# vr308/Generalised-Gaussian-Processes

Hardware: AMD Instinct MI355X
Metric: ELBO evals/sec (higher is better)
Workload: dtype f64

## Files before the change

### generalised-gaussian-processes_amd/_lib.py

```python
from __future__ import annotations

import ctypes as C
import os

HERE = os.path.dirname(os.path.abspath(__file__))
LIB_PATH = os.path.join(HERE, "csrc", "libsgp_hip.so")

SGP_ABI_VERSION = 3
SGP_MAX_DIM = 32
SGP_MAX_INDUCING = 4096
KERNEL_IDS = {"rbf": 0, "matern32": 1, "matern52": 2, "composite": 3}
LIKELIHOOD_IDS = {"gaussian": 0, "bernoulli": 1, "bernoulli_logit": 2, "poisson": 3}
SGPMC_LIK_OUT_LEN = 3
SGP_LIK_MULTICLASS_ROBUSTMAX = 4
SGP_MAX_CLASSES = 16
COMP_LEN = 33
OPT_CONTRACTION, OPT_ASM_OVERLAP, OPT_KFU_BUDGET_BYTES, OPT_COND_LIMIT, OPT_CU_BUDGET, OPT_TIMING, OPT_SHARED_DEVICE = range(7)
OUT_F, OUT_LOGMARG, OUT_TRACE, OUT_LOGDETB, OUT_QUAD, OUT_TRW, OUT_S2BAR, OUT_KAPPABAR, OUT_LEN = range(9)


class SgpLibraryError(RuntimeError):
    pass


class SgpStatusError(RuntimeError):
    def __init__(self, fn, status, text):
        super().__init__("%s returned %d: %s" % (fn, status, text))
        self.status = status


_vp, _i64, _i32, _dbl, _sz = C.c_void_p, C.c_int64, C.c_int, C.c_double, C.c_size_t
_dp = C.POINTER(C.c_double)
# ... 329 lines not shown
```

### generalised-gaussian-processes_amd/core.py

```python
from __future__ import annotations

import math

import torch

try:
    import torch.distributed as dist
except Exception:
    dist = None

from ._lib import COMP_LEN, OUT_F, OUT_LOGMARG, OUT_S2BAR, OUT_TRACE


class NotPositiveDefiniteError(RuntimeError):

    def __init__(self, info):
        super().__init__("matrix not positive definite: leading minor of order %d (1..M: Kuu, M+1..2M: B)" % info)
        self.info = info


class SgpTimeoutError(RuntimeError):

    def __init__(self):
        super().__init__("device time-out inside the dataflow Cholesky (SGP_INFO_TIMEOUT): outputs are invalid")
# ... 346 lines not shown
            self._allreduce_stats(packed, M)
            kw = {"want_cw": True} if factored else {}
            res = e.bound(Kuu, packed, s2, self.N, with_adjoints=with_adjoints, want_factors=want_factors, kuu_linv=linv,
                          result=result, whitened=True, **kw)
            if rep:
                e.streaming_error_report(None, 1, self._trace_buf(), sf2, s2, self.N, M, result)
                res["reported"] = True
            res.update(packed=packed, kfu=None, t_keep=t_keep, linv=linv)
            return res
        kfu = self._kfu_for(M) if with_adjoints else None
        gate = None
        guard = report
        trace = self._trace_buf() if guard and hasattr(e, "kuu_factor") else None
        overlap = (self.overlap_tail and hasattr(e, "kuu_factor") and e.device.type == "cuda"
                   and int(self.X.shape[0]) * M >= self.overlap_min_work)
        if overlap:
            main = torch.cuda.current_stream(e.device)
            side, (z_ready, ready), (Kuu, linv) = self._side_state(M)
            z_ready.record(main)
            side.wait_event(z_ready)
            e.kuu(Z, ls, sf2, self.jitter, self.kernel, out=Kuu, stream=side)
            e.kuu_factor(Kuu, info=result[2], trace_out=trace, out=linv, stream=side)
            ready.record(side)
            if (hasattr(e, "would_use_i8") and self.kernel != "composite" and int(self.X.shape[0]) >= 300 * M
                    and e.would_use_i8(int(self.X.shape[0]), M)):
                gate = ready
        try:
            packed = e.suffstats(self.X, self.y, Z, ls, sf2, self.kernel, kfu=kfu, **({"gate": gate} if gate is not None else {}))
            self._allreduce_stats(packed, M)
        finally:
            if overlap:
                main.wait_event(ready)
        if overlap:
            res = e.bound(Kuu, packed, s2, self.N, with_adjoints=with_adjoints, want_factors=want_factors, kuu_linv=linv,
                          result=result)
        elif guard and hasattr(e, "kuu_factor"):
            Kuu = e.kuu(Z, ls, sf2, self.jitter, self.kernel)
            linv, _ = e.kuu_factor(Kuu, info=result[2], trace_out=trace)
            res = e.bound(Kuu, packed, s2, self.N, with_adjoints=with_adjoints, want_factors=want_factors, kuu_linv=linv,
                          result=result)
        else:
            Kuu = e.kuu(Z, ls, sf2, self.jitter, self.kernel)
            res = e.bound(Kuu, packed, s2, self.N, with_adjoints=with_adjoints, want_factors=want_factors, result=result)
        if guard and trace is not None:
            e.streaming_error_report(packed, M + 1, trace, sf2, s2, self.N, M, result)
            res["reported"] = True
        res["packed"] = packed
        res["kfu"] = kfu
        return res

    def _pass2(self, res, Z, ls, sf2, s2, want_gz, g):
        e = self.engine
        if res.get("Cw") is not None:
            e.suffstats_bwd_factored(self.X, self.y, Z, ls, sf2, res["linv"], res["Cw"], s2, res["bbar"], -1.0 / (2.0 * float(s2)),
                                     self.kernel, want_gz=want_gz, out=g,
                                     **({"t_in": res["t_keep"]} if res.get("t_keep") is not None else {}))
        else:
            e.suffstats_bwd(self.X, self.y, Z, ls, sf2, res["Phibar"], res["bbar"], -1.0 / (2.0 * float(s2)),
                            self.kernel, want_gz=want_gz, out=g, kfu=res["kfu"])
            if res.get("Phibar_lo") is not None:
# ... 180 lines not shown
```

### generalised-gaussian-processes_amd/csrc/sgp_ctx.hip

```cpp
#include "sgp_common.hpp"
#include "sgp_ctx.hpp"
#include "sgp_stream.hpp"
#include <cstdlib>
#include <new>

namespace sgp {

static void ctx_init(Ctx& c, int device) {
  c.device = device;
  c.contraction = env_int("SGP_CONTRACTION", 1);
  if (c.contraction < 0 || c.contraction > 2) c.contraction = 1;
  c.asm_overlap = env_int("SGP_ASM_OVERLAP", 0);
  c.kfu_budget = KFU_BUDGET_DEFAULT;
  c.syrk_skip_upper = env_int("SGP_SYRK_SKIP_UPPER", 1);
  c.syrk_waves = env_int("SGP_SYRK_WAVES", 4);
  c.syrk_glds = env_int("SGP_SYRK_GLDS", 0);
  c.i8_prio = env_int("SGP_I8_PRIO", 0);
  c.shared_device = env_int("SGP_SHARED_DEVICE", 0) != 0 ? 1 : 0;
}

Ctx& default_ctx() {
  static Ctx* c = [] {
    Ctx* p = new Ctx();
    int dev = 0;
    if (hipGetDevice(&dev) != hipSuccess) dev = 0;
    ctx_init(*p, dev);
    return p;
  }();
  return *c;
}

static thread_local Ctx* t_cur = nullptr;
static thread_local Ctx* t_bound = nullptr;
// ... 51 lines not shown
      if (!(value >= 0.0)) return SGP_ERR_ARG;
      c.kfu_budget = value > 0.0 ? (size_t)value : KFU_BUDGET_DEFAULT;
      return SGP_OK;
    case SGP_OPT_COND_LIMIT:
      c.cond_limit = value >= 0.0 ? value : 1e13;
      return SGP_OK;
    case SGP_OPT_CU_BUDGET:
      c.cu_budget = value > 0.0 ? (int)value : 0;
      return SGP_OK;
    case SGP_OPT_TIMING:
      c.timing = value != 0.0 ? 1 : 0;
      return SGP_OK;
    case SGP_OPT_SHARED_DEVICE:
      c.shared_device = value != 0.0 ? 1 : 0;
      return SGP_OK;
    default:
      return SGP_ERR_ARG;
  }
}

extern "C" double sgp_ctx_get_option(const sgp_ctx* ctx, int option) {
  const Ctx& c = ctx ? *reinterpret_cast<const Ctx*>(ctx) : default_ctx();
  switch (option) {
    case SGP_OPT_CONTRACTION: return (double)c.contraction;
    case SGP_OPT_ASM_OVERLAP: return (double)c.asm_overlap;
    case SGP_OPT_KFU_BUDGET_BYTES: return (double)c.kfu_budget;
    case SGP_OPT_COND_LIMIT: return c.cond_limit;
    case SGP_OPT_CU_BUDGET: return (double)c.cu_budget;
    case SGP_OPT_TIMING: return (double)c.timing;
    case SGP_OPT_SHARED_DEVICE: return (double)c.shared_device;
    default: return -1.0;
  }
}

extern "C" void sgp_ctx_bind_thread(sgp_ctx* ctx) { sgp::bind_thread_ctx(ctx); }

extern "C" int sgp_ctx_device(const sgp_ctx* ctx) { return (ctx ? *reinterpret_cast<const Ctx*>(ctx) : default_ctx()).device; }

extern "C" void sgp_ctx_set_pass1_gate(sgp_ctx* ctx, void* hip_event) {
  (ctx ? *reinterpret_cast<Ctx*>(ctx) : default_ctx()).pass1_gate = (hipEvent_t)hip_event;
}

extern "C" int sgp_ctx_contraction_last(const sgp_ctx* ctx) {
  return (ctx ? *reinterpret_cast<const Ctx*>(ctx) : default_ctx()).contraction_used;
}
// ... 159 lines not shown
```

### generalised-gaussian-processes_amd/csrc/sgp_ctx.hpp

```cpp
#pragma once
#include <hip/hip_runtime.h>
#include <cstddef>
#include <cstdint>

namespace sgp {

constexpr int CTX_TIMING_SLOTS = 3;

struct Ctx {
  int device = 0;
  int contraction = 1;
  int asm_overlap = 0;
  size_t kfu_budget = 0;
  double cond_limit = 1e13;
  int cu_budget = 0;
  int timing = 0;
  int shared_device = 0;
  int syrk_skip_upper = 1, syrk_waves = 4, syrk_glds = 0, i8_prio = 0;
  int contraction_used = 0;
  hipEvent_t pass1_gate = nullptr;
  int64_t syrk_timed_rows = 0;
  hipEvent_t ev[CTX_TIMING_SLOTS][2] = {};
  int ev_ready = 0, ev_used[CTX_TIMING_SLOTS] = {0, 0, 0};
  hipStream_t side = nullptr;
  hipEvent_t ev_fork = nullptr, ev_join = nullptr;
};

Ctx& default_ctx();
Ctx& cur_ctx();

void bind_thread_ctx(void* ctx);

struct CtxScope {
  Ctx* prev;
  explicit CtxScope(void* ctx);
// ... 7 lines not shown
```

### generalised-gaussian-processes_amd/csrc/sgp_suffstats_fwd.hip

```cpp
#include "sgp_common.hpp"
#include "sgp_stream.hpp"
#include "sgp_dense.hpp"
#include "sgp_composite.hpp"
#include "sgp_ctx.hpp"
#include <cstdlib>

namespace sgp {

static_assert(TIMING_SLOTS == CTX_TIMING_SLOTS, "timing slots");
size_t stream_kfu_budget() { return cur_ctx().kfu_budget; }

void timing_begin(int slot, hipStream_t st) {
  Ctx& c = cur_ctx();
  if (!c.timing) return;
  if (!c.ev_ready) {
    bool ok = true;
    for (int s = 0; s < TIMING_SLOTS; ++s)
      for (int k = 0; k < 2; ++k) ok = (hipEventCreate(&c.ev[s][k]) == hipSuccess) && ok;
    if (!ok) return;
    c.ev_ready = 1;
  }
  if (hipEventRecord(c.ev[slot][0], st) != hipSuccess) c.ev_used[slot] = 0;
}
void timing_end(int slot, hipStream_t st) {
// ... 304 lines not shown
    split = (nsplit & ~7) + u / ntiles;
  }
  int ti = (int)((sqrt(8.0 * t + 1.0) - 1.0) * 0.5);
  while ((ti + 1) * (ti + 2) / 2 <= t) ++ti;
  while (ti * (ti + 1) / 2 > t) --ti;
  const int tj = t - ti * (ti + 1) / 2;
  int64_t c0, c1;
  split_range(smap, split, nchunks, c0, c1);
  double* out = slab + ((size_t)split * ntiles + t) * (TILE * TILE);
  if (ti == tj)
    syrk_tile<true, NW, GLDS, SKIP>(Ks, Kfu, Mp, c0, c1, ti * TILE, tj * TILE, accumulate, out);
  else
    syrk_tile<false, NW, GLDS, SKIP>(Ks, Kfu, Mp, c0, c1, ti * TILE, tj * TILE, accumulate, out);
}

__global__ __launch_bounds__(256) void reduce_phi_kernel(const double* __restrict__ slab, int nsplit, int ntiles,
                                                         int M, double scale, double* __restrict__ Phi) {
  __shared__ double tile[32][33];
  const int t = blockIdx.x;
  int bi = (int)((sqrt(8.0 * t + 1.0) - 1.0) * 0.5);
  while ((bi + 1) * (bi + 2) / 2 <= t) ++bi;
  while (bi * (bi + 1) / 2 > t) --bi;
  const int bj = t - bi * (bi + 1) / 2;
  const int tx = threadIdx.x & 31, ty = threadIdx.x >> 5;
  const int Ti = (bi * 32) / TILE, Tj = (bj * 32) / TILE;
  const int tileidx = Ti * (Ti + 1) / 2 + Tj;
  const double* base = slab + (size_t)tileidx * (TILE * TILE);
  const size_t sstride = (size_t)ntiles * (TILE * TILE);
#pragma unroll
  for (int k = 0; k < 4; ++k) {
    const int lr = ty + 8 * k;
    const int gi = bi * 32 + lr, gj = bj * 32 + tx;
    double s = 0.0;
    if (gi >= gj) {
      const size_t off = (size_t)(gi - Ti * TILE) * TILE + (gj - Tj * TILE);
#pragma unroll 8
      for (int sp = 0; sp < nsplit; ++sp) s += base[sp * sstride + off];
    }
    tile[lr][tx] = s * scale;
  }
  __syncthreads();
#pragma unroll
  for (int k = 0; k < 4; ++k) {
    const int lr = ty + 8 * k;
    const int gi = bi * 32 + lr, gj = bj * 32 + tx;
    if (gi < M && gj < M && gi >= gj) Phi[(size_t)gi * M + gj] = tile[lr][tx];
    const int mi = bj * 32 + lr, mj = bi * 32 + tx;
    if (mi < M && mj < M && mj > mi) Phi[(size_t)mi * M + mj] = tile[tx][lr];
  }
}

__global__ __launch_bounds__(256) void bpart_stage1_kernel(const double* __restrict__ bpart, int64_t nrb, int Mp, int G,
                                                           double* __restrict__ tmp) {
  __shared__ double part[4][64];
  const int col = blockIdx.x * 64 + (threadIdx.x & 63), w = threadIdx.x >> 6, g = blockIdx.y;
  double s = 0.0;
  for (int64_t rb = g + (int64_t)w * G; rb < nrb; rb += 4 * (int64_t)G) s += bpart[rb * Mp + col];
  part[w][threadIdx.x & 63] = s;
  __syncthreads();
  if (w == 0) {
    const int l = threadIdx.x;
    tmp[(size_t)g * Mp + col] = (part[0][l] + part[1][l]) + (part[2][l] + part[3][l]);
  }
}
// ... 4 lines not shown
                                                             double* __restrict__ yy, double* __restrict__ kappa) {
  const int m = blockIdx.x * 256 + threadIdx.x;
  if (m < M) {
    double s = 0.0;
#pragma unroll 8
    for (int g = 0; g < G; ++g) s += btmp[(size_t)g * Mp + m];
    b[m] = s * sf2;
  }
  if (blockIdx.x == 0) {
    __shared__ double red[4];
    double s = 0.0;
    for (int i = threadIdx.x; i < nyy; i += 256) s += yypart[i];
    s = block_sum256(s, red);
    if (threadIdx.x == 0) {
      *yy = s;
      *kappa = kappa_val;
    }
  }
}

template <int DP, int ROWS>
static void launch_assemble_rows(int kid, dim3 grid, hipStream_t st, const double* Xs, const double* ys, const double* Zs,
                                 int64_t row0, int64_t N, int M, int Mp, double* Kfu, double* bpart) {
  switch (kid) {
    case SGP_KERNEL_RBF: kfu_assemble_kernel<DP, SGP_KERNEL_RBF, ROWS><<<grid, 256, 0, st>>>(Xs, ys, Zs, row0, N, M, Mp, Kfu, bpart); break;
    case SGP_KERNEL_MATERN32: kfu_assemble_kernel<DP, SGP_KERNEL_MATERN32, ROWS><<<grid, 256, 0, st>>>(Xs, ys, Zs, row0, N, M, Mp, Kfu, bpart); break;
    default: kfu_assemble_kernel<DP, SGP_KERNEL_MATERN52, ROWS><<<grid, 256, 0, st>>>(Xs, ys, Zs, row0, N, M, Mp, Kfu, bpart); break;
  }
}
template <int DP>
// ... 110 lines not shown
                   double* b, double* yy, double* kappa, hipStream_t st) {
  bpart_stage1_kernel<<<dim3(p.Mp / 64, BRED_G), 256, 0, st>>>(bpart, p.Npad / ASM_ROWS * nparts, p.Mp, BRED_G, btmp);
  finalize_stats_kernel<<<(M + 255) / 256, 256, 0, st>>>(btmp, BRED_G, p.Mp, M, yypart, 256, sf2, sf2 * (double)N, b, yy, kappa);
}
template <typename Ws>
static void finish_b(const StreamPlan& p, const Ws& w, int nparts, double sf2, int64_t N, int M, double* b, double* yy, double* kappa,
                     hipStream_t st) {
  reduce_bparts(p, w.bpart, w.btmp, w.yypart, nparts, sf2, N, M, b, yy, kappa, st);
}
void reduce_slabs(const StreamPlan& p, const double* slab, int nslabs, int M, double scale, double* Phi, hipStream_t st) {
  const int nb32 = p.Mp / 32;
  reduce_phi_kernel<<<nb32 * (nb32 + 1) / 2, 256, 0, st>>>(slab, nslabs, p.ntiles, M, scale, Phi);
}
static void finish_stats(const StreamPlan& p, const FwdWs& w, int nslabs, int nparts, double sf2, int64_t N, int M, double* Phi, double* b,
                         double* yy, double* kappa, hipStream_t st) {
  reduce_slabs(p, w.slab, nslabs, M, sf2 * sf2, Phi, st);
  finish_b(p, w, nparts, sf2, N, M, b, yy, kappa, st);
}

__global__ __launch_bounds__(256) void tpart_kernel(const double* __restrict__ T, const double* __restrict__ ys, int64_t row0, int Mp,
                                                    double* __restrict__ bpart) {
  __shared__ double ysh[ASM_ROWS];
  const int64_t rbase = (int64_t)blockIdx.x * ASM_ROWS;
  ysh[threadIdx.x] = ys[row0 + rbase + threadIdx.x];
  __syncthreads();
  const int m = blockIdx.y * 256 + threadIdx.x;
  if (m >= Mp) return;
  const double* src = T + (size_t)rbase * Mp + m;
  double a0 = 0.0, a1 = 0.0, a2 = 0.0, a3 = 0.0;
#pragma unroll 2
// ... 470 lines not shown
```

### generalised-gaussian-processes_amd/csrc/sgp_tail.hip

```cpp
#include "sgp_dense.hpp"
#include "sgp_ctx.hpp"
#include "sgp_composite.hpp"
#include "sgp_stream.hpp"

namespace sgp {

template <int KID>
__global__ __launch_bounds__(256) void kuu_kernel(const double* __restrict__ Z, int64_t ldz, KernArgs ka, double jitter,
                                                  int M, double* __restrict__ Kuu) {
  const int64_t total = (int64_t)M * M;
  for (int64_t e = (int64_t)blockIdx.x * 256 + threadIdx.x; e < total; e += (int64_t)gridDim.x * 256) {
    const int i = (int)(e / M), j = (int)(e - (int64_t)i * M);
    double r2 = 0.0;
    for (int q = 0; q < ka.d; ++q) {
      const double df = (Z[i * ldz + q] - Z[j * ldz + q]) * ka.inv_ls[q];
      r2 = fma(df, df, r2);
    }
    double v = ka.sf2 * kprofile<KID>(r2);
    if (i == j) v += jitter;
    Kuu[e] = v;
  }
}

template <int KID>
// ... 121 lines not shown
        else g_ls[q] += -2.0 * ka.inv_ls[q] * s;
      }
    }
  }
  if (g_Z) {
    const int64_t total = (int64_t)M * d;
    for (int64_t e = (int64_t)blockIdx.x * 256 + threadIdx.x; e < total; e += (int64_t)gridDim.x * 256) {
      const int q = (int)(e % d);
      g_Z[e] += 4.0 * ka.inv_ls[q] * gzraw[e];
    }
  }
}

enum { SC_TRW = 0, SC_LOGDET = 1, SC_QQ = 2, SC_TRSP = 3, SC_BA = 4, SC_APA = 5, SC_N = 8 };

__global__ __launch_bounds__(256) void make_B_kernel(const double* __restrict__ W, int Mp, double inv_s2, double* __restrict__ Bm,
                                                     double* __restrict__ trW, double* __restrict__ zero_me, int nB,
                                                     const double* __restrict__ Li, const double* __restrict__ x, double* __restrict__ y) {
  if ((int)blockIdx.x >= nB) {
    const int row = ((int)blockIdx.x - nB) * 4 + (threadIdx.x >> 6), lane = threadIdx.x & 63;
    if (row >= Mp) return;
    double s = 0.0;
    for (int j = lane; j < Mp; j += 64) s = fma(Li[(int64_t)row * Mp + j], x[j], s);
    s = wave_sum(s);
    if (lane == 0) y[row] = s;
    return;
  }
  const int64_t total = (int64_t)Mp * Mp;
  for (int64_t e = (int64_t)blockIdx.x * 256 + threadIdx.x; e < total; e += (int64_t)nB * 256) {
    const int r = (int)(e / Mp), c = (int)(e - (int64_t)r * Mp);
    const double w = 0.5 * (W[e] + W[(int64_t)c * Mp + r]);
    Bm[e] = (r == c ? 1.0 : 0.0) + w * inv_s2;
    if (zero_me) zero_me[e] = 0.0;
  }
  if ((int)blockIdx.x == nB - 1) {
    __shared__ double red[4];
    double s = 0.0;
    for (int i = threadIdx.x; i < Mp; i += 256) s += W[(int64_t)i * Mp + i];
// ... 76 lines not shown
  out[SGP_OUT_LOGMARG] = logmarg;
  out[SGP_OUT_TRACE] = trace_term;
  out[SGP_OUT_LOGDETB] = logdetB;
  out[SGP_OUT_QUAD] = quad;
  out[SGP_OUT_TRW] = trW;
  if (with_adj) {
    const double s22 = s2 * s2;
    out[SGP_OUT_S2BAR] = -0.5 * (-trSP / s22 + Nd / s2 - *yy / s22 + 2.0 * ba / (s22 * s2) - aPa / (s22 * s22)
                                 - *kappa / s22 + trW / s22);
    out[SGP_OUT_KAPPABAR] = -1.0 / (2.0 * s2);
  } else {
    out[SGP_OUT_S2BAR] = 0.0;
    out[SGP_OUT_KAPPABAR] = 0.0;
  }
}
__global__ __launch_bounds__(256) void finalize_bound_kernel(FinalizeArgs a) {
  __shared__ double red[4];
  finalize_bound_body(a, red);
}

__global__ __launch_bounds__(1024) void adjoint_mid_kernel(const double* __restrict__ W, const double* __restrict__ Binv,
                                                           const double* __restrict__ g, const double* __restrict__ u,
                                                           const double* __restrict__ Li, int Mp, double s2, int nC,
                                                           double* __restrict__ CS, double* __restrict__ rows3, double* __restrict__ t) {
  __shared__ double part[16][64];
  const int b = blockIdx.x, lane = threadIdx.x & 63, wv = threadIdx.x >> 6;
  if (b < nC) {
    const int64_t total = (int64_t)Mp * Mp;
    const double is2 = 1.0 / s2, is22 = 1.0 / (s2 * s2);
    for (int64_t e = (int64_t)b * 1024 + threadIdx.x; e < total; e += (int64_t)nC * 1024) {
      const int r = (int)(e / Mp), c = (int)(e - (int64_t)r * Mp);
      const int64_t pt = (int64_t)c * Mp + r;
      const double w = 0.5 * (W[e] + W[pt]);
// ... 34 lines not shown
      s3 = fma(Li[(int64_t)(j + 48) * Mp + col], g[j + 48], s3);
    }
    for (; j < Mp; j += 16) s0 = fma(Li[(int64_t)j * Mp + col], g[j], s0);
    part[wv][lane] = (s0 + s1) + (s2_ + s3);
    __syncthreads();
    if (wv == 0) {
      double acc = 0.0;
#pragma unroll
      for (int k = 0; k < 16; ++k) acc += part[k][lane];
      t[col] = acc;
    }
  }
}
__global__ __launch_bounds__(256) void adjoint_out_kernel(const double* __restrict__ R, const double* __restrict__ t,
                                                          int Mp, int M, double s2, double* __restrict__ Phibar,
                                                          double* __restrict__ Kuubar, double* __restrict__ bbar, int nA, FinalizeArgs fin) {
  if ((int)blockIdx.x == nA) {
    __shared__ double red[4];
    finalize_bound_body(fin, red);
    return;
  }
  const int64_t total = (int64_t)M * M;
  const int64_t mm = (int64_t)Mp * Mp;
  const double h = 0.25 / s2;
  for (int64_t e = (int64_t)blockIdx.x * 256 + threadIdx.x; e < total; e += (int64_t)nA * 256) {
    const int r = (int)(e / M), c = (int)(e - (int64_t)r * M);
    const int64_t p = (int64_t)r * Mp + c, pt = (int64_t)c * Mp + r;
    Phibar[e] = h * (R[p] + R[pt]);
    Kuubar[e] = -0.25 * (R[mm + p] + R[mm + pt]);
  }
  const double is22 = 1.0 / (s2 * s2);
  if (blockIdx.x == 0)
    for (int i = threadIdx.x; i < M; i += 256) bbar[i] = t[i] * is22;
}
// ... 452 lines not shown
}

__global__ void streaming_bound_kernel(const double* __restrict__ tr, double sf2, double s2, double* __restrict__ est) {
  est[0] = 0x1p-53 * sf2 * sf2 * tr[0] / s2;
}
extern "C" int sgp_streaming_error_bound(const double* trace_inv, double sf2, double s2, double* est, sgp_stream_t stream) {
  if (!trace_inv || !est || !(s2 > 0.0) || !(sf2 > 0.0)) return SGP_ERR_ARG;
  streaming_bound_kernel<<<1, 1, 0, (hipStream_t)stream>>>(trace_inv, sf2, s2, est);
  return check_launch();
}

__global__ __launch_bounds__(256) void streaming_report_kernel(const double* __restrict__ diag, int64_t stride, int M,
                                                               const double* __restrict__ tr, double sf2, double s2, double n,
                                                               double* __restrict__ est) {
  __shared__ double red[4];
  double mx = 0.0;
  if (diag)
    for (int i = threadIdx.x; i < M; i += 256) mx = fmax(mx, diag[(int64_t)i * stride]);
#pragma unroll
  for (int o = 32; o > 0; o >>= 1) mx = fmax(mx, __shfl_xor(mx, o, 64));
  if ((threadIdx.x & 63) == 0) red[threadIdx.x >> 6] = mx;
  __syncthreads();
  if (threadIdx.x == 0) {
    const double ub = 0x1p-53 * sf2 * sf2 * tr[0] / s2;
    est[1] = ub;
    est[0] = diag ? 0x1p-53 * fmax(fmax(red[0], red[1]), fmax(red[2], red[3])) * tr[0] / (s2 * n) : ub;
  }
}
extern "C" int sgp_streaming_error_report(const double* diag, int64_t stride, const double* trace_inv, double sf2, double s2, int64_t N,
                                          int M, double* est, sgp_stream_t stream) {
  if (!trace_inv || !est || M <= 0 || N < 0 || !(s2 > 0.0) || !(sf2 > 0.0) || (diag && stride <= 0)) return SGP_ERR_ARG;
  if (M > SGP_MAX_INDUCING) return SGP_ERR_DIM;
  streaming_report_kernel<<<1, 256, 0, (hipStream_t)stream>>>(diag, stride, M, trace_inv, sf2, s2, N > 0 ? (double)N : 1.0, est);
  return check_launch();
}

extern "C" void sgp_set_cond_limit(double limit) { default_ctx().cond_limit = limit >= 0.0 ? limit : 1e13; }

static int bound_impl(const double* Kuu, const double* Phi, const double* b, const double* yy,
                      const double* kappa, double s2, int64_t N, int M, int with_adjoints, double* out,
                      double* Phibar, double* bbar, double* Kuubar, double* factors,
                      const double* kuu_linv, int* info, void* ws, size_t ws_bytes,
                      sgp_stream_t stream, bool whitened, double* Cw_out = nullptr) {
  if ((!Kuu && !kuu_linv) || !Phi || !b || !yy || !kappa || !out || !info || M <= 0 || N < 0 || !(s2 > 0.0)) return SGP_ERR_ARG;
  if (whitened && !kuu_linv) return SGP_ERR_ARG;
  if (with_adjoints && (!Phibar || !bbar || !Kuubar)) return SGP_ERR_ARG;
  if (M > SGP_MAX_INDUCING) return SGP_ERR_DIM;
  const int Mp = padded_m(M);
  BoundWs w = carve_bound(ws, Mp, 1);
  if (!ws || ws_bytes < w.bytes) return SGP_ERR_WORKSPACE;
  hipStream_t st = (hipStream_t)stream;
  const int64_t ld = Mp;
  const size_t mm = (size_t)Mp * Mp;
  const bool need_G = with_adjoints || factors;

  const int nflags = (int)potrf_flag_ints(Mp);
  tail_prep_kernel<<<(nflags + 255) / 256, 256, 0, st>>>(kuu_linv ? nullptr : info, w.sc, w.flagsB, nflags, b, M, Mp, w.bp);

  if (kuu_linv) {
    w.M1 = const_cast<double*>(kuu_linv);
  } else {
    pad_copy(Kuu, M, M, M, w.M0, ld, Mp, Mp, 1.0, st);
    if (!potrf_lower(w.M0, w.M1, ld, Mp, info, 0, w.flags, st)) tri_inverse(w.M0, w.M1, w.M2, ld, Mp, st);
  }

  if (whitened) {
    if (M == Mp) w.M5 = const_cast<double*>(Phi);
    else pad_copy(Phi, M, M, M, w.M5, ld, Mp, Mp, 0.0, st);
    w.u = w.bp;
  } else {
  if (M == Mp) w.M3 = const_cast<double*>(Phi);
  else pad_copy(Phi, M, M, M, w.M3, ld, Mp, Mp, 0.0, st);
// ... 3 lines not shown
    g.m = Mp; g.n = Mp; g.k = Mp; g.khi_mask = 1;
    g.lower_only = true;
    gemm(g, st);
    GemmDesc h;
    h.A = w.M4; h.lda = ld; h.B = w.M1; h.ldb = ld; h.tb = true; h.C = w.M5; h.ldc = ld;
    h.m = Mp; h.n = Mp; h.k = Mp; h.khi_mask = 2;
    h.lower_only = true;
    h.mirror = true;
    gemm(h, st);
  }

  }

  {
    const int nB = grid_for((int64_t)mm);
    make_B_kernel<<<nB + (whitened ? 0 : Mp / 4), 256, 0, st>>>(w.M5, Mp, 1.0 / s2, w.M6, w.sc + SC_TRW, need_G ? w.M7 : nullptr, nB, w.M1,
                                                                w.bp, w.u);
  }
  const bool lb_inverted = potrf_lower(w.M6, need_G ? w.M7 : nullptr, ld, Mp, info, M, w.flagsB, st, w.u, w.q, true, 2);
  const int* abort_flag = potrf_abort_flag(w.flagsB, Mp);
  if (need_G && !lb_inverted) tri_inverse(w.M6, w.M7, w.M2, ld, Mp, st);

  if (factors) {
    crop_copy(w.M1, ld, factors, M, M, M, st);
    crop_copy(w.M7, ld, factors + (size_t)M * M, M, M, M, st);
    crop_copy(w.q, 1, factors + (size_t)2 * M * M, 1, M, 1, st);
  }
  if (with_adjoints) {
    GemmDesc s;
    s.A = w.M7; s.lda = ld; s.ta = true; s.B = w.M7; s.ldb = ld; s.C = w.M2; s.ldc = ld;
    s.m = Mp; s.n = Mp; s.k = Mp; s.klo_mask = 3;
    gemm(s, st);
// ... 5 lines not shown
      adjoint_mid_kernel<<<nC + Mp / 16 + Mp / 64, 1024, 0, st>>>(w.M5, w.M2, w.alpha, w.u, w.M1, Mp, s2, nC, CS, w.rows3, w.t1);
    }
    if (Cw_out) crop_copy(CS, ld, Cw_out, M, M, M, st);
    GemmDesc t1;
    t1.A = CS; t1.lda = ld; t1.sA = (int64_t)mm; t1.B = w.M1; t1.ldb = ld; t1.sB = 0; t1.C = TT; t1.ldc = ld; t1.sC = (int64_t)mm;
    t1.m = Mp; t1.n = Mp; t1.k = Mp; t1.batch = 2; t1.klo_mask = 2;
    gemm(t1, st);
    GemmDesc t2;
    t2.A = w.M1; t2.lda = ld; t2.ta = true; t2.sA = 0; t2.B = TT; t2.ldb = ld; t2.sB = (int64_t)mm; t2.C = CS; t2.ldc = ld; t2.sC = (int64_t)mm;
    t2.m = Mp; t2.n = Mp; t2.k = Mp; t2.batch = 2; t2.klo_mask = 1;
    gemm(t2, st);
  }
  const FinalizeArgs fin{w.sc, yy, kappa, s2, (double)N, with_adjoints, w.M6, w.q, Mp, abort_flag, info, out, w.rows3};
  if (with_adjoints) {
    const int nA = grid_for((int64_t)M * M);
    adjoint_out_kernel<<<nA + 1, 256, 0, st>>>(w.M0, w.t1, Mp, M, s2, Phibar, Kuubar, bbar, nA, fin);
  } else {
    finalize_bound_kernel<<<1, 256, 0, st>>>(fin);
  }
  return check_launch();
}

extern "C" int sgp_bound_from_stats(const double* Kuu, const double* Phi, const double* b, const double* yy,
                                    const double* kappa, double s2, int64_t N, int M, int with_adjoints, double* out,
                                    double* Phibar, double* bbar, double* Kuubar, double* factors,
                                    const double* kuu_linv, int* info, void* ws, size_t ws_bytes,
                                    sgp_stream_t stream) {
  return bound_impl(Kuu, Phi, b, yy, kappa, s2, N, M, with_adjoints, out, Phibar, bbar, Kuubar, factors, kuu_linv, info, ws,
                    ws_bytes, stream, false);
}
extern "C" int sgp_bound_from_whitened_stats(const double* W, const double* u, const double* yy, const double* kappa, double s2,
// ... 190 lines not shown
```

### generalised-gaussian-processes_amd/engine.py

```python
from __future__ import annotations

import ctypes as C
from typing import Optional, Sequence

import numpy as np
import torch

from . import _lib
from ._lib import COMP_LEN, KERNEL_IDS, OUT_LEN

RESULT_HEAD = OUT_LEN + 4


def _kernel_id(kernel) -> int:
    if isinstance(kernel, int):
        if kernel not in KERNEL_IDS.values():
            raise ValueError("unknown kernel id %r" % (kernel,))
        return kernel
    try:
        return KERNEL_IDS[str(kernel).lower()]
    except KeyError:
        raise ValueError("unknown kernel %r (expected one of %s)" % (kernel, sorted(KERNEL_IDS))) from None


# ... 5 lines not shown


_F64 = torch.float64


def _chk(device, t: torch.Tensor, name: str) -> torch.Tensor:
    if t.dtype is not _F64 or t.device != device or not t.is_contiguous():
        raise ValueError("%s must be a contiguous float64 tensor on %s (got %s, %s)" % (name, device, t.dtype, t.device))
    return t


class HipEngine:

    OPTIONS = {"contraction": _lib.OPT_CONTRACTION, "asm_overlap": _lib.OPT_ASM_OVERLAP, "kfu_budget_bytes": _lib.OPT_KFU_BUDGET_BYTES,
               "cond_limit": _lib.OPT_COND_LIMIT, "cu_budget": _lib.OPT_CU_BUDGET, "timing": _lib.OPT_TIMING,
               "shared_device": _lib.OPT_SHARED_DEVICE}

    def __init__(self, device: Optional[torch.device] = None, own_context: bool = False):
        self.lib = _lib.load_library()
        if not torch.cuda.is_available():
            raise _lib.SgpLibraryError("HipEngine needs a HIP device (torch.cuda.is_available() is False); "
                                       "there is no CPU implementation of the sparse-GP core")
        self.device = torch.device(device) if device is not None else torch.device("cuda", torch.cuda.current_device())
        self._ws = {}
        self._ctx = None
        if own_context:
            self._ctx = self.lib.sgp_ctx_create(self.device.index if self.device.index is not None else torch.cuda.current_device())
            if not self._ctx:
                raise _lib.SgpLibraryError("sgp_ctx_create failed")

    def __del__(self):
# ... 101 lines not shown
            self._chk(X, "X"), self._chk(y, "y")
        if out is None:
            out = self.empty(M * M + M + 2)
        nbytes = ws_query(self._c(), N, M, d, *query_args)
        if nbytes == 0:
            raise ValueError("unsupported shape N=%d M=%d d=%d%s" % (N, M, d, limits))
        base = out.data_ptr()
        stats = [C.c_void_p(base + 8 * o) for o in (0, M * M, M * M + M, M * M + M + 1)]
        return N, M, d, out, self._workspace(ws_name, nbytes), stats

    def kfu_buffer(self, N: int, M: int) -> torch.Tensor:
        return self.empty(self.lib.sgp_kfu_len(N, M))

    def kfu_f16_buffer(self, N: int, M: int) -> torch.Tensor:
        return torch.empty(self.lib.sgp_kfu_len(N, M), dtype=torch.float16, device=self.device)

    def suffstats(self, X, y, Z, ls, sf2, kernel="rbf", out: Optional[torch.Tensor] = None,
                  kfu: Optional[torch.Tensor] = None, gate: Optional[torch.cuda.Event] = None) -> torch.Tensor:
        N, M, d, out, ws, stats = self._pass1(X, y, Z, None, out, "fwd_kfu" if kfu is not None else "fwd",
                                              self.lib.sgp_ctx_suffstats_workspace_bytes, 1 if kfu is not None else 0,
                                              limits=" (d <= %d, M <= %d)" % (_lib.SGP_MAX_DIM, _lib.SGP_MAX_INDUCING))
        if gate is not None:
            self.lib.sgp_ctx_set_pass1_gate(self._c(), C.c_void_p(gate.cuda_event))
        st = self.lib.sgp_ctx_suffstats_fwd(
            self._c(), self._ptr(X), d, self._ptr(y), self._ptr(Z), d, self._inv_ls(ls, d, kernel), float(sf2), N, M, d, _kernel_id(kernel),
            *stats, self._ptr(kfu), self._ptr(ws), ws.numel(), self._stream())
        _lib.check("sgp_suffstats_fwd", st)
        return out

    def suffstats_whitened(self, X, y, Z, ls, sf2, kuu_linv, kernel="rbf", out: Optional[torch.Tensor] = None) -> torch.Tensor:
# ... 121 lines not shown
        return out

    def streaming_error_estimate(self, packed, trace, s2, N, M, result) -> None:
        buf = result[0]
        est = C.c_void_p(buf.data_ptr() + 8 * (OUT_LEN + 1))
        _lib.check("sgp_streaming_error_estimate",
                   self.lib.sgp_streaming_error_estimate(self._ptr(packed), self._ptr(trace), float(s2), int(N), int(M), est, self._stream()))

    def streaming_error_bound(self, trace, sf2, s2, result) -> None:
        est = C.c_void_p(result[0].data_ptr() + 8 * (OUT_LEN + 1))
        _lib.check("sgp_streaming_error_bound", self.lib.sgp_streaming_error_bound(self._ptr(trace), float(sf2), float(s2), est, self._stream()))

    def streaming_error_report(self, diag, stride, trace, sf2, s2, N, M, result) -> None:
        est = C.c_void_p(result[0].data_ptr() + 8 * (OUT_LEN + 1))
        _lib.check("sgp_streaming_error_report",
                   self.lib.sgp_streaming_error_report(self._ptr(diag), int(stride), self._ptr(trace),
                                                       float(sf2), float(s2), int(N), int(M), est, self._stream()))

    @staticmethod
    def read_estimate(host_buf) -> float:
        return float(host_buf[OUT_LEN + 1])

    @staticmethod
    def read_bound(host_buf) -> float:
        return float(host_buf[OUT_LEN + 2])

    def bound(self, Kuu, packed, s2, N, with_adjoints=False, want_factors=False, kuu_linv=None, kuu_info=None, result=None,
              whitened=False, want_cw=False):
        M = Kuu.shape[0]
        self._chk(Kuu, "Kuu"), self._chk(packed, "packed")
        if whitened and kuu_linv is None:
            raise ValueError("bound(whitened=True) needs kuu_linv (the factor the statistics were whitened with)")
        buf, out, info = result if result is not None else self.result_buffer()
        if kuu_linv is not None:
            if kuu_info is not None:
                info.copy_(kuu_info)
            elif result is None:
                raise ValueError("bound(kuu_linv=...) needs the status of kuu_factor: kuu_info= or result=")
        res = {"out": out, "info": info, "buf": buf}
        Phibar = bbar = Kuubar = factors = None
        if with_adjoints:
            Phibar, bbar, Kuubar = self.empty(M, M), self.empty(M), self.empty(M, M)
            res.update(Phibar=Phibar, bbar=bbar, Kuubar=Kuubar)
        if want_factors:
            factors = self.empty(self.lib.sgp_bound_factors_len(M))
            res["factors"] = factors
        nbytes = self.lib.sgp_bound_workspace_bytes(M, 1 if with_adjoints else 0)
        ws = self._workspace("bound", nbytes)
        base = packed.data_ptr()
        stats = (C.c_void_p(base), C.c_void_p(base + 8 * M * M), C.c_void_p(base + 8 * (M * M + M)),
                 C.c_void_p(base + 8 * (M * M + M + 1)))
        tail = (float(s2), int(N), M, 1 if with_adjoints else 0, self._ptr(out), self._ptr(Phibar), self._ptr(bbar),
                self._ptr(Kuubar), self._ptr(factors), self._ptr(kuu_linv), self._ptr(info), self._ptr(ws), ws.numel(), self._stream())
        if whitened:
            if want_cw and with_adjoints:
                res["Cw"] = self.empty(M, M)
            _lib.check("sgp_bound_from_whitened_stats",
                       self.lib.sgp_ctx_bound_from_whitened_stats(self._c(), *stats, *tail[:-3], self._ptr(res.get("Cw")), *tail[-3:]))
        else:
            _lib.check("sgp_bound_from_stats", self.lib.sgp_ctx_bound_from_stats(self._c(), self._ptr(Kuu), *stats, *tail))
        return res

    def sgpmc_tail(self, packed_whitened, v, s2, N, kuu_linv, with_adjoints=False, result=None, vbar_out=None):
        M = int(v.numel())
        self._chk(packed_whitened, "packed_whitened"), self._chk(v, "v")
        if packed_whitened.numel() < M * M + M + 2:
            raise ValueError("packed_whitened holds %d doubles, M * M + M + 2 = %d" % (packed_whitened.numel(), M * M + M + 2))
        buf, out, info = result if result is not None else self.result_buffer()
# ... 913 lines not shown
```

### include/sgp.h

```cpp
#ifndef SGP_H
#define SGP_H

#include <stddef.h>
#include <stdint.h>

#ifdef __cplusplus
extern "C" {
#endif
#if defined(__GNUC__) || defined(__clang__)
#pragma GCC visibility push(default)
#endif

typedef void* sgp_stream_t;

#define SGP_ABI_VERSION 3
#define SGP_MAX_DIM 32
#define SGP_MAX_INDUCING 4096

#define SGP_INFO_TIMEOUT (-7777)

#define SGP_KERNEL_RBF 0
#define SGP_KERNEL_MATERN32 1
#define SGP_KERNEL_MATERN52 2
#define SGP_KERNEL_COMPOSITE 3
// ... 20 lines not shown
#define SGP_OUT_TRW 5
#define SGP_OUT_S2BAR 6
#define SGP_OUT_KAPPABAR 7
#define SGP_OUT_LEN 8

int sgp_abi_version(void);

typedef struct sgp_ctx sgp_ctx;
#define SGP_OPT_CONTRACTION 0
#define SGP_OPT_ASM_OVERLAP 1
#define SGP_OPT_KFU_BUDGET_BYTES 2
#define SGP_OPT_COND_LIMIT 3
#define SGP_OPT_CU_BUDGET 4
#define SGP_OPT_TIMING 5
#define SGP_OPT_SHARED_DEVICE 6
sgp_ctx* sgp_ctx_create(int device);
void sgp_ctx_destroy(sgp_ctx* ctx);
int sgp_ctx_device(const sgp_ctx* ctx);
int sgp_ctx_set_option(sgp_ctx* ctx, int option, double value);
double sgp_ctx_get_option(const sgp_ctx* ctx, int option);
void sgp_ctx_bind_thread(sgp_ctx* ctx);
void sgp_ctx_set_pass1_gate(sgp_ctx* ctx, void* hip_event);
int sgp_ctx_contraction_last(const sgp_ctx* ctx);
int sgp_ctx_contraction_would_use_i8(const sgp_ctx* ctx, int64_t N, int M);
int sgp_ctx_timing_last_ms(sgp_ctx* ctx, int slot, float* ms);
int64_t sgp_ctx_timing_last_rows(const sgp_ctx* ctx, int slot);
size_t sgp_ctx_suffstats_workspace_bytes(const sgp_ctx* ctx, int64_t N, int M, int d, int caller_owns_kfu);
int sgp_ctx_suffstats_fwd(sgp_ctx* ctx, const double* X, int64_t ldx, const double* y, const double* Z, int64_t ldz,
                          const double* inv_ls, double sf2, int64_t N, int M, int d, int kernel_id, double* Phi, double* b,
                          double* yy, double* kappa, double* Kfu_out, void* ws, size_t ws_bytes, sgp_stream_t stream);
// ... 377 lines not shown
```

Before: 71.35.

## Fuse pass-1 close-out, tail prep and error report into fewer kernel launches

Merges the Phi slab reduction and the b/yy/kappa reduction into one pass1_closeout kernel. Folds the tail_prep zeroing work into extra blocks of make_B when a Kuu inverse is supplied. Defers the streaming error report so it runs as an extra block of the finalize or adjoint_out kernel. Together these remove several small launches and their serialization from the ELBO tail, at the cost of new context state for the deferred report and more kernels with mixed roles. Everything sits behind a tail_fused option that defaults on.

```diff
diff --git a/generalised-gaussian-processes_amd/_lib.py b/generalised-gaussian-processes_amd/_lib.py
--- a/generalised-gaussian-processes_amd/_lib.py
+++ b/generalised-gaussian-processes_amd/_lib.py
@@ -16,6 +16,7 @@
 SGP_MAX_CLASSES = 16
 COMP_LEN = 33
 OPT_CONTRACTION, OPT_ASM_OVERLAP, OPT_KFU_BUDGET_BYTES, OPT_COND_LIMIT, OPT_CU_BUDGET, OPT_TIMING, OPT_SHARED_DEVICE = range(7)
+OPT_TAIL_FUSED, OPT_REPORT_DEFER = 7, 8
 OUT_F, OUT_LOGMARG, OUT_TRACE, OUT_LOGDETB, OUT_QUAD, OUT_TRW, OUT_S2BAR, OUT_KAPPABAR, OUT_LEN = range(9)
 
 
diff --git a/generalised-gaussian-processes_amd/core.py b/generalised-gaussian-processes_amd/core.py
--- a/generalised-gaussian-processes_amd/core.py
+++ b/generalised-gaussian-processes_amd/core.py
@@ -384,6 +384,7 @@
         trace = self._trace_buf() if guard and hasattr(e, "kuu_factor") else None
         overlap = (self.overlap_tail and hasattr(e, "kuu_factor") and e.device.type == "cuda"
                    and int(self.X.shape[0]) * M >= self.overlap_min_work)
+        fused = hasattr(e, "tail_fused") and e.tail_fused()
         if overlap:
             main = torch.cuda.current_stream(e.device)
             side, (z_ready, ready), (Kuu, linv) = self._side_state(M)
@@ -401,19 +402,21 @@
         finally:
             if overlap:
                 main.wait_event(ready)
+        rep = {"report": (packed, M + 1, trace, sf2)} if (fused and guard and trace is not None) else {}
         if overlap:
             res = e.bound(Kuu, packed, s2, self.N, with_adjoints=with_adjoints, want_factors=want_factors, kuu_linv=linv,
-                          result=result)
+                          result=result, **rep)
         elif guard and hasattr(e, "kuu_factor"):
             Kuu = e.kuu(Z, ls, sf2, self.jitter, self.kernel)
             linv, _ = e.kuu_factor(Kuu, info=result[2], trace_out=trace)
             res = e.bound(Kuu, packed, s2, self.N, with_adjoints=with_adjoints, want_factors=want_factors, kuu_linv=linv,
-                          result=result)
+                          result=result, **rep)
         else:
             Kuu = e.kuu(Z, ls, sf2, self.jitter, self.kernel)
             res = e.bound(Kuu, packed, s2, self.N, with_adjoints=with_adjoints, want_factors=want_factors, result=result)
         if guard and trace is not None:
-            e.streaming_error_report(packed, M + 1, trace, sf2, s2, self.N, M, result)
+            if not rep:
+                e.streaming_error_report(packed, M + 1, trace, sf2, s2, self.N, M, result)
             res["reported"] = True
         res["packed"] = packed
         res["kfu"] = kfu
diff --git a/generalised-gaussian-processes_amd/csrc/sgp_ctx.hip b/generalised-gaussian-processes_amd/csrc/sgp_ctx.hip
--- a/generalised-gaussian-processes_amd/csrc/sgp_ctx.hip
+++ b/generalised-gaussian-processes_amd/csrc/sgp_ctx.hip
@@ -17,6 +17,7 @@
   c.syrk_glds = env_int("SGP_SYRK_GLDS", 0);
   c.i8_prio = env_int("SGP_I8_PRIO", 0);
   c.shared_device = env_int("SGP_SHARED_DEVICE", 0) != 0 ? 1 : 0;
+  c.tail_fused = env_int("SGP_TAIL_FUSED", 1) != 0 ? 1 : 0;
 }
 
 Ctx& default_ctx() {
@@ -98,6 +99,12 @@
     case SGP_OPT_SHARED_DEVICE:
       c.shared_device = value != 0.0 ? 1 : 0;
       return SGP_OK;
+    case SGP_OPT_TAIL_FUSED:
+      c.tail_fused = value != 0.0 ? 1 : 0;
+      return SGP_OK;
+    case SGP_OPT_REPORT_DEFER:
+      c.report_defer = value != 0.0 ? 1 : 0;
+      return SGP_OK;
     default:
       return SGP_ERR_ARG;
   }
@@ -113,6 +120,8 @@
     case SGP_OPT_CU_BUDGET: return (double)c.cu_budget;
     case SGP_OPT_TIMING: return (double)c.timing;
     case SGP_OPT_SHARED_DEVICE: return (double)c.shared_device;
+    case SGP_OPT_TAIL_FUSED: return (double)c.tail_fused;
+    case SGP_OPT_REPORT_DEFER: return (double)c.report_defer;
     default: return -1.0;
   }
 }
diff --git a/generalised-gaussian-processes_amd/csrc/sgp_ctx.hpp b/generalised-gaussian-processes_amd/csrc/sgp_ctx.hpp
--- a/generalised-gaussian-processes_amd/csrc/sgp_ctx.hpp
+++ b/generalised-gaussian-processes_amd/csrc/sgp_ctx.hpp
@@ -16,9 +16,19 @@
   int cu_budget = 0;
   int timing = 0;
   int shared_device = 0;
+  int tail_fused = 1;
   int syrk_skip_upper = 1, syrk_waves = 4, syrk_glds = 0, i8_prio = 0;
   int contraction_used = 0;
   hipEvent_t pass1_gate = nullptr;
+  int report_defer = 0, report_pending = 0;
+  struct {
+    const double* diag;
+    int64_t stride;
+    int M;
+    const double* tr;
+    double sf2, s2, n;
+    double* est;
+  } report = {};
   int64_t syrk_timed_rows = 0;
   hipEvent_t ev[CTX_TIMING_SLOTS][2] = {};
   int ev_ready = 0, ev_used[CTX_TIMING_SLOTS] = {0, 0, 0};
diff --git a/generalised-gaussian-processes_amd/csrc/sgp_suffstats_fwd.hip b/generalised-gaussian-processes_amd/csrc/sgp_suffstats_fwd.hip
--- a/generalised-gaussian-processes_amd/csrc/sgp_suffstats_fwd.hip
+++ b/generalised-gaussian-processes_amd/csrc/sgp_suffstats_fwd.hip
@@ -342,10 +342,8 @@
     syrk_tile<false, NW, GLDS, SKIP>(Ks, Kfu, Mp, c0, c1, ti * TILE, tj * TILE, accumulate, out);
 }
 
-__global__ __launch_bounds__(256) void reduce_phi_kernel(const double* __restrict__ slab, int nsplit, int ntiles,
-                                                         int M, double scale, double* __restrict__ Phi) {
-  __shared__ double tile[32][33];
-  const int t = blockIdx.x;
+__device__ __forceinline__ void reduce_phi_block(const double* __restrict__ slab, int nsplit, int ntiles, int M, double scale,
+                                                 double* __restrict__ Phi, int t, double (*tile)[33]) {
   int bi = (int)((sqrt(8.0 * t + 1.0) - 1.0) * 0.5);
   while ((bi + 1) * (bi + 2) / 2 <= t) ++bi;
   while (bi * (bi + 1) / 2 > t) --bi;
@@ -376,6 +374,11 @@
     const int mi = bj * 32 + lr, mj = bi * 32 + tx;
     if (mi < M && mj < M && mj > mi) Phi[(size_t)mi * M + mj] = tile[tx][lr];
   }
+}
+__global__ __launch_bounds__(256) void reduce_phi_kernel(const double* __restrict__ slab, int nsplit, int ntiles,
+                                                         int M, double scale, double* __restrict__ Phi) {
+  __shared__ double tile[32][33];
+  reduce_phi_block(slab, nsplit, ntiles, M, scale, Phi, blockIdx.x, tile);
 }
 
 __global__ __launch_bounds__(256) void bpart_stage1_kernel(const double* __restrict__ bpart, int64_t nrb, int Mp, int G,
@@ -410,6 +413,52 @@
     s = block_sum256(s, red);
     if (threadIdx.x == 0) {
       *yy = s;
+      *kappa = kappa_val;
+    }
+  }
+}
+
+constexpr int CLOSE_COLS = 16, CLOSE_G = 64;
+__global__ __launch_bounds__(256) void pass1_closeout_kernel(const double* __restrict__ slab, int nsplit, int ntiles, int M, double scale,
+                                                             double* __restrict__ Phi, int nbb, const double* __restrict__ bpart,
+                                                             int64_t nrb, int Mp, const double* __restrict__ yypart, int nyy, double sf2,
+                                                             double kappa_val, double* __restrict__ b, double* __restrict__ yy,
+                                                             double* __restrict__ kappa) {
+  __shared__ double sm[4 * CLOSE_G * CLOSE_COLS];
+  if ((int)blockIdx.x >= nbb) {
+    reduce_phi_block(slab, nsplit, ntiles, M, scale, Phi, (int)blockIdx.x - nbb, reinterpret_cast<double (*)[33]>(sm));
+    return;
+  }
+  double (*part)[CLOSE_G][CLOSE_COLS] = reinterpret_cast<double (*)[CLOSE_G][CLOSE_COLS]>(sm);
+  const int c0 = blockIdx.x * CLOSE_COLS, g = threadIdx.x & 63, w = threadIdx.x >> 6;
+  double s[CLOSE_COLS];
+#pragma unroll
+  for (int c = 0; c < CLOSE_COLS; ++c) s[c] = 0.0;
+  for (int64_t rb = g + (int64_t)w * CLOSE_G; rb < nrb; rb += 4 * (int64_t)CLOSE_G) {
+    const double* row = bpart + rb * Mp + c0;
+#pragma unroll
+    for (int c = 0; c < CLOSE_COLS; ++c) s[c] += row[c];
+  }
+#pragma unroll
+  for (int c = 0; c < CLOSE_COLS; ++c) part[w][g][c] = s[c];
+  __syncthreads();
+  for (int e = threadIdx.x; e < CLOSE_G * CLOSE_COLS; e += 256) {
+    const int gg = e / CLOSE_COLS, c = e - gg * CLOSE_COLS;
+    part[0][gg][c] = (part[0][gg][c] + part[1][gg][c]) + (part[2][gg][c] + part[3][gg][c]);
+  }
+  __syncthreads();
+  if ((int)threadIdx.x < CLOSE_COLS && c0 + (int)threadIdx.x < M) {
+    double t = 0.0;
+    for (int gg = 0; gg < CLOSE_G; ++gg) t += part[0][gg][threadIdx.x];
+    b[c0 + threadIdx.x] = t * sf2;
+  }
+  if (blockIdx.x == 0) {
+    __shared__ double red[4];
+    double t = 0.0;
+    for (int i = threadIdx.x; i < nyy; i += 256) t += yypart[i];
+    t = block_sum256(t, red);
+    if (threadIdx.x == 0) {
+      *yy = t;
       *kappa = kappa_val;
     }
   }
@@ -550,6 +599,14 @@
 }
 static void finish_stats(const StreamPlan& p, const FwdWs& w, int nslabs, int nparts, double sf2, int64_t N, int M, double* Phi, double* b,
                          double* yy, double* kappa, hipStream_t st) {
+  static_assert(CLOSE_G == BRED_G, "the fused close-out walks the two-stage b reduction's groups");
+  if (cur_ctx().tail_fused) {
+    const int nb32 = p.Mp / 32, nbb = p.Mp / CLOSE_COLS;
+    pass1_closeout_kernel<<<nbb + nb32 * (nb32 + 1) / 2, 256, 0, st>>>(w.slab, nslabs, p.ntiles, M, sf2 * sf2, Phi, nbb, w.bpart,
+                                                                        p.Npad / ASM_ROWS * nparts, p.Mp, w.yypart, 256, sf2,
+                                                                        sf2 * (double)N, b, yy, kappa);
+    return;
+  }
   reduce_slabs(p, w.slab, nslabs, M, sf2 * sf2, Phi, st);
   finish_b(p, w, nparts, sf2, N, M, b, yy, kappa, st);
 }
diff --git a/generalised-gaussian-processes_amd/csrc/sgp_tail.hip b/generalised-gaussian-processes_amd/csrc/sgp_tail.hip
--- a/generalised-gaussian-processes_amd/csrc/sgp_tail.hip
+++ b/generalised-gaussian-processes_amd/csrc/sgp_tail.hip
@@ -159,14 +159,29 @@
 
 enum { SC_TRW = 0, SC_LOGDET = 1, SC_QQ = 2, SC_TRSP = 3, SC_BA = 4, SC_APA = 5, SC_N = 8 };
 
+struct TailPrep {
+  int nblk;
+  double* sc;
+  int* flags;
+  int nflags;
+  double* bp;
+};
 __global__ __launch_bounds__(256) void make_B_kernel(const double* __restrict__ W, int Mp, double inv_s2, double* __restrict__ Bm,
                                                      double* __restrict__ trW, double* __restrict__ zero_me, int nB,
-                                                     const double* __restrict__ Li, const double* __restrict__ x, double* __restrict__ y) {
+                                                     const double* __restrict__ Li, const double* __restrict__ x, double* __restrict__ y,
+                                                     int nG, int xM, TailPrep prep) {
+  if ((int)blockIdx.x >= nB + nG) {
+    const int e0 = ((int)blockIdx.x - nB - nG) * 256 + threadIdx.x, stride = prep.nblk * 256;
+    if (e0 < SC_N && e0 != SC_TRW) prep.sc[e0] = 0.0;
+    for (int e = e0; e < prep.nflags; e += stride) prep.flags[e] = 0;
+    for (int e = e0; e < Mp; e += stride) prep.bp[e] = e < xM ? x[e] : 0.0;
+    return;
+  }
   if ((int)blockIdx.x >= nB) {
     const int row = ((int)blockIdx.x - nB) * 4 + (threadIdx.x >> 6), lane = threadIdx.x & 63;
     if (row >= Mp) return;
     double s = 0.0;
-    for (int j = lane; j < Mp; j += 64) s = fma(Li[(int64_t)row * Mp + j], x[j], s);
+    for (int j = lane; j < Mp; j += 64) s = fma(Li[(int64_t)row * Mp + j], j < xM ? x[j] : 0.0, s);
     s = wave_sum(s);
     if (lane == 0) y[row] = s;
     return;
@@ -273,9 +288,38 @@
     out[SGP_OUT_KAPPABAR] = 0.0;
   }
 }
+struct ReportArgs {
+  const double* diag;
+  int64_t stride;
+  int M;
+  const double* tr;
+  double sf2, s2, n;
+  double* est;
+};
+__device__ __forceinline__ void streaming_report_body(const ReportArgs& r, double* red) {
+  const double* __restrict__ diag = r.diag;
+  const double* __restrict__ tr = r.tr;
+  double mx = 0.0;
+  if (diag)
+    for (int i = threadIdx.x; i < r.M; i += 256) mx = fmax(mx, diag[(int64_t)i * r.stride]);
+#pragma unroll
+  for (int o = 32; o > 0; o >>= 1) mx = fmax(mx, __shfl_xor(mx, o, 64));
+  if ((threadIdx.x & 63) == 0) red[threadIdx.x >> 6] = mx;
+  __syncthreads();
+  if (threadIdx.x == 0) {
+    const double ub = 0x1p-53 * r.sf2 * r.sf2 * tr[0] / r.s2;
+    r.est[1] = ub;
+    r.est[0] = diag ? 0x1p-53 * fmax(fmax(red[0], red[1]), fmax(red[2], red[3])) * tr[0] / (r.s2 * r.n) : ub;
+  }
+}
 __global__ __launch_bounds__(256) void finalize_bound_kernel(FinalizeArgs a) {
   __shared__ double red[4];
   finalize_bound_body(a, red);
+}
+__global__ __launch_bounds__(256) void finalize_report_kernel(FinalizeArgs a, ReportArgs r) {
+  __shared__ double red[4];
+  if (blockIdx.x == 0) finalize_bound_body(a, red);
+  else streaming_report_body(r, red);
 }
 
 __global__ __launch_bounds__(1024) void adjoint_mid_kernel(const double* __restrict__ W, const double* __restrict__ Binv,
@@ -340,10 +384,12 @@
 }
 __global__ __launch_bounds__(256) void adjoint_out_kernel(const double* __restrict__ R, const double* __restrict__ t,
                                                           int Mp, int M, double s2, double* __restrict__ Phibar,
-                                                          double* __restrict__ Kuubar, double* __restrict__ bbar, int nA, FinalizeArgs fin) {
-  if ((int)blockIdx.x == nA) {
+                                                          double* __restrict__ Kuubar, double* __restrict__ bbar, int nA, FinalizeArgs fin,
+                                                          ReportArgs rep) {
+  if ((int)blockIdx.x >= nA) {
     __shared__ double red[4];
-    finalize_bound_body(fin, red);
+    if ((int)blockIdx.x == nA) finalize_bound_body(fin, red);
+    else streaming_report_body(rep, red);
     return;
   }
   const int64_t total = (int64_t)M * M;
@@ -826,23 +872,20 @@
                                                                const double* __restrict__ tr, double sf2, double s2, double n,
                                                                double* __restrict__ est) {
   __shared__ double red[4];
-  double mx = 0.0;
-  if (diag)
-    for (int i = threadIdx.x; i < M; i += 256) mx = fmax(mx, diag[(int64_t)i * stride]);
-#pragma unroll
-  for (int o = 32; o > 0; o >>= 1) mx = fmax(mx, __shfl_xor(mx, o, 64));
-  if ((threadIdx.x & 63) == 0) red[threadIdx.x >> 6] = mx;
-  __syncthreads();
-  if (threadIdx.x == 0) {
-    const double ub = 0x1p-53 * sf2 * sf2 * tr[0] / s2;
-    est[1] = ub;
-    est[0] = diag ? 0x1p-53 * fmax(fmax(red[0], red[1]), fmax(red[2], red[3])) * tr[0] / (s2 * n) : ub;
-  }
+  streaming_report_body(ReportArgs{diag, stride, M, tr, sf2, s2, n, est}, red);
 }
 extern "C" int sgp_streaming_error_report(const double* diag, int64_t stride, const double* trace_inv, double sf2, double s2, int64_t N,
                                           int M, double* est, sgp_stream_t stream) {
+  Ctx& cx = cur_ctx();
+  const bool defer = cx.report_defer != 0 && cx.tail_fused != 0;
+  cx.report_defer = 0;
   if (!trace_inv || !est || M <= 0 || N < 0 || !(s2 > 0.0) || !(sf2 > 0.0) || (diag && stride <= 0)) return SGP_ERR_ARG;
   if (M > SGP_MAX_INDUCING) return SGP_ERR_DIM;
+  if (defer) {
+    cx.report = {diag, stride, M, trace_inv, sf2, s2, N > 0 ? (double)N : 1.0, est};
+    cx.report_pending = 1;
+    return SGP_OK;
+  }
   streaming_report_kernel<<<1, 256, 0, (hipStream_t)stream>>>(diag, stride, M, trace_inv, sf2, s2, N > 0 ? (double)N : 1.0, est);
   return check_launch();
 }
@@ -854,6 +897,10 @@
                       double* Phibar, double* bbar, double* Kuubar, double* factors,
                       const double* kuu_linv, int* info, void* ws, size_t ws_bytes,
                       sgp_stream_t stream, bool whitened, double* Cw_out = nullptr) {
+  Ctx& cx = cur_ctx();
+  ReportArgs rep{};
+  if (cx.report_pending) rep = ReportArgs{cx.report.diag, cx.report.stride, cx.report.M, cx.report.tr, cx.report.sf2, cx.report.s2, cx.report.n, cx.report.est};
+  cx.report_pending = 0;
   if ((!Kuu && !kuu_linv) || !Phi || !b || !yy || !kappa || !out || !info || M <= 0 || N < 0 || !(s2 > 0.0)) return SGP_ERR_ARG;
   if (whitened && !kuu_linv) return SGP_ERR_ARG;
   if (with_adjoints && (!Phibar || !bbar || !Kuubar)) return SGP_ERR_ARG;
@@ -867,7 +914,8 @@
   const bool need_G = with_adjoints || factors;
 
   const int nflags = (int)potrf_flag_ints(Mp);
-  tail_prep_kernel<<<(nflags + 255) / 256, 256, 0, st>>>(kuu_linv ? nullptr : info, w.sc, w.flagsB, nflags, b, M, Mp, w.bp);
+  const bool fused = cx.tail_fused != 0, prep_fused = fused && kuu_linv != nullptr;
+  if (!prep_fused) tail_prep_kernel<<<(nflags + 255) / 256, 256, 0, st>>>(kuu_linv ? nullptr : info, w.sc, w.flagsB, nflags, b, M, Mp, w.bp);
 
   if (kuu_linv) {
     w.M1 = const_cast<double*>(kuu_linv);
@@ -901,8 +949,15 @@
 
   {
     const int nB = grid_for((int64_t)mm);
-    make_B_kernel<<<nB + (whitened ? 0 : Mp / 4), 256, 0, st>>>(w.M5, Mp, 1.0 / s2, w.M6, w.sc + SC_TRW, need_G ? w.M7 : nullptr, nB, w.M1,
-                                                                w.bp, w.u);
+    const int nG = whitened ? 0 : Mp / 4;
+    if (prep_fused) {
+      const TailPrep prep{(nflags + 255) / 256, w.sc, w.flagsB, nflags, w.bp};
+      make_B_kernel<<<nB + nG + prep.nblk, 256, 0, st>>>(w.M5, Mp, 1.0 / s2, w.M6, w.sc + SC_TRW, need_G ? w.M7 : nullptr, nB, w.M1, b, w.u,
+                                                         nG, M, prep);
+    } else {
+      make_B_kernel<<<nB + nG, 256, 0, st>>>(w.M5, Mp, 1.0 / s2, w.M6, w.sc + SC_TRW, need_G ? w.M7 : nullptr, nB, w.M1, w.bp, w.u, nG, Mp,
+                                             TailPrep{});
+    }
   }
   const bool lb_inverted = potrf_lower(w.M6, need_G ? w.M7 : nullptr, ld, Mp, info, M, w.flagsB, st, w.u, w.q, true, 2);
   const int* abort_flag = potrf_abort_flag(w.flagsB, Mp);
@@ -938,7 +993,9 @@
   const FinalizeArgs fin{w.sc, yy, kappa, s2, (double)N, with_adjoints, w.M6, w.q, Mp, abort_flag, info, out, w.rows3};
   if (with_adjoints) {
     const int nA = grid_for((int64_t)M * M);
-    adjoint_out_kernel<<<nA + 1, 256, 0, st>>>(w.M0, w.t1, Mp, M, s2, Phibar, Kuubar, bbar, nA, fin);
+    adjoint_out_kernel<<<nA + 1 + (rep.est ? 1 : 0), 256, 0, st>>>(w.M0, w.t1, Mp, M, s2, Phibar, Kuubar, bbar, nA, fin, rep);
+  } else if (rep.est) {
+    finalize_report_kernel<<<2, 256, 0, st>>>(fin, rep);
   } else {
     finalize_bound_kernel<<<1, 256, 0, st>>>(fin);
   }
diff --git a/generalised-gaussian-processes_amd/engine.py b/generalised-gaussian-processes_amd/engine.py
--- a/generalised-gaussian-processes_amd/engine.py
+++ b/generalised-gaussian-processes_amd/engine.py
@@ -43,7 +43,7 @@
 
     OPTIONS = {"contraction": _lib.OPT_CONTRACTION, "asm_overlap": _lib.OPT_ASM_OVERLAP, "kfu_budget_bytes": _lib.OPT_KFU_BUDGET_BYTES,
                "cond_limit": _lib.OPT_COND_LIMIT, "cu_budget": _lib.OPT_CU_BUDGET, "timing": _lib.OPT_TIMING,
-               "shared_device": _lib.OPT_SHARED_DEVICE}
+               "shared_device": _lib.OPT_SHARED_DEVICE, "tail_fused": _lib.OPT_TAIL_FUSED}
 
     def __init__(self, device: Optional[torch.device] = None, own_context: bool = False):
         self.lib = _lib.load_library()
@@ -175,6 +175,9 @@
 
     def kfu_f16_buffer(self, N: int, M: int) -> torch.Tensor:
         return torch.empty(self.lib.sgp_kfu_len(N, M), dtype=torch.float16, device=self.device)
+
+    def tail_fused(self) -> bool:
+        return self.get_option("tail_fused") != 0
 
     def suffstats(self, X, y, Z, ls, sf2, kernel="rbf", out: Optional[torch.Tensor] = None,
                   kfu: Optional[torch.Tensor] = None, gate: Optional[torch.cuda.Event] = None) -> torch.Tensor:
@@ -326,7 +329,7 @@
     def streaming_error_report(self, diag, stride, trace, sf2, s2, N, M, result) -> None:
         est = C.c_void_p(result[0].data_ptr() + 8 * (OUT_LEN + 1))
         _lib.check("sgp_streaming_error_report",
-                   self.lib.sgp_streaming_error_report(self._ptr(diag), int(stride), self._ptr(trace),
+                   self._cf.sgp_streaming_error_report(self._ptr(diag), int(stride), self._ptr(trace),
                                                        float(sf2), float(s2), int(N), int(M), est, self._stream()))
 
     @staticmethod
@@ -338,7 +341,7 @@
         return float(host_buf[OUT_LEN + 2])
 
     def bound(self, Kuu, packed, s2, N, with_adjoints=False, want_factors=False, kuu_linv=None, kuu_info=None, result=None,
-              whitened=False, want_cw=False):
+              whitened=False, want_cw=False, report=None):
         M = Kuu.shape[0]
         self._chk(Kuu, "Kuu"), self._chk(packed, "packed")
         if whitened and kuu_linv is None:
@@ -364,6 +367,9 @@
                  C.c_void_p(base + 8 * (M * M + M + 1)))
         tail = (float(s2), int(N), M, 1 if with_adjoints else 0, self._ptr(out), self._ptr(Phibar), self._ptr(bbar),
                 self._ptr(Kuubar), self._ptr(factors), self._ptr(kuu_linv), self._ptr(info), self._ptr(ws), ws.numel(), self._stream())
+        if report is not None:
+            self.lib.sgp_ctx_set_option(self._c(), _lib.OPT_REPORT_DEFER, 1.0)
+            self.streaming_error_report(report[0], report[1], report[2], report[3], s2, N, M, (buf, out, info))
         if whitened:
             if want_cw and with_adjoints:
                 res["Cw"] = self.empty(M, M)
diff --git a/include/sgp.h b/include/sgp.h
--- a/include/sgp.h
+++ b/include/sgp.h
@@ -58,6 +58,8 @@
 #define SGP_OPT_CU_BUDGET 4
 #define SGP_OPT_TIMING 5
 #define SGP_OPT_SHARED_DEVICE 6
+#define SGP_OPT_TAIL_FUSED 7
+#define SGP_OPT_REPORT_DEFER 8
 sgp_ctx* sgp_ctx_create(int device);
 void sgp_ctx_destroy(sgp_ctx* ctx);
 int sgp_ctx_device(const sgp_ctx* ctx);
```

Result: no change. 71.24 (-0.2%).
